# JunyiPeng00/wespeaker_hubert

Measured on AMD Instinct MI355X. Metric: embeddings/sec on 5s 16kHz utts, higher is better.
Workload: dtype f32 (bf16x3 split MFMA, fp32 accumulate)

## Files before the change

### wespeaker_hubert_amd/csrc/conv_gemm_x3_t6.hip

```cpp
#include "conv_gemm_x3_g.h"

namespace wsp {
namespace {

constexpr int kGCsLd = 68;
constexpr int kGCsBytes = 8 * 64 * kGCsLd * 4;
template <int ACT>
__device__ __forceinline__ void g_epilogue_cs(const ConvGemmArgs& p, f32x4 (&acc)[4][8], int m0, int n0, int wm,
                                              int wn, int wave, int lane, unsigned char* smem) {
  float* stg = reinterpret_cast<float*>(smem) + wave * 64 * kGCsLd;
  const int c16 = lane & 15, q = lane >> 4;
  const int cl = 4 * c16;
  const __amdgpu_buffer_rsrc_t ro = make_rsrc(p.out);
  const int nb = min((m0 / p.T + 1) * p.T, p.M) - m0, mb = p.M - m0;
  unsigned side0 = 0, side1 = 0;
#pragma unroll
  for (int k = 0; k < 16; ++k) {
    const int rr = wm * 64 + (k >> 2) * 16 + 4 * q + (k & 3);
    side0 |= (rr < nb ? 1u : 0u) << k;
    side1 |= (rr >= nb && rr < mb ? 1u : 0u) << k;
  }
  double rs[8][2];
#pragma unroll
  for (int pp = 0; pp < 2; ++pp) {
#pragma unroll
    for (int i = 0; i < 4; ++i)
#pragma unroll
      for (int jj = 0; jj < 4; ++jj)
#pragma unroll
        for (int r = 0; r < 4; ++r) stg[(16 * i + 4 * q + r) * kGCsLd + 16 * jj + c16] = acc[i][4 * pp + jj][r];
    asm volatile("s_waitcnt lgkmcnt(0)" ::: "memory");
    const int col = n0 + wn * 128 + 64 * pp + cl;
    const f32x4 bv = p.bias ? *reinterpret_cast<const f32x4*>(p.bias + col) : f32x4{0.f, 0.f, 0.f, 0.f};
    const f32x4 sc = p.scale ? *reinterpret_cast<const f32x4*>(p.scale + col) : f32x4{1.f, 1.f, 1.f, 1.f};
    const f32x4 sh = p.scale ? *reinterpret_cast<const f32x4*>(p.shift + col) : f32x4{0.f, 0.f, 0.f, 0.f};
#pragma unroll
    for (int u = 0; u < 16; ++u) {
      const int rl = 4 * u + q;
      const int row = m0 + wm * 64 + rl;
      float* sp = stg + rl * kGCsLd + cl;
      const f32x4 x = *reinterpret_cast<const f32x4*>(sp);
      f32x4 y;
#pragma unroll
      for (int e = 0; e < 4; ++e) {
        float v = x[e] + bv[e];
        if constexpr (ACT == kActRelu) v = fmaxf(v, 0.f);
        else if constexpr (ACT == kActTanh) v = tanhf(v);
        else if constexpr (ACT == kActGelu) v = gelu_as(v);
        y[e] = v * sc[e] + sh[e];
      }
      __builtin_amdgcn_raw_buffer_store_b128(__builtin_bit_cast(u32x4, y), ro,
                                             row < p.M ? (row * p.ldo + col) * 4 : kOOB, 0, 0);
      *reinterpret_cast<f32x4*>(sp) = y;
    }
    asm volatile("s_waitcnt lgkmcnt(0)" ::: "memory");
#pragma unroll
    for (int jj = 0; jj < 4; ++jj) {
      double c0 = 0.0, c1 = 0.0;
#pragma unroll
      for (int k = 0; k < 16; ++k) {
        const double yd = (double)stg[((k >> 2) * 16 + 4 * q + (k & 3)) * kGCsLd + 16 * jj + c16];
        c0 += (side0 >> k) & 1 ? yd : 0.0;
        c1 += (side1 >> k) & 1 ? yd : 0.0;
      }
      double v0 = c0 + __shfl_xor(c0, 16);
      v0 += __shfl_xor(v0, 32);
      double v1 = c1 + __shfl_xor(c1, 16);
      v1 += __shfl_xor(v1, 32);
      rs[4 * pp + jj][0] = v0;
      rs[4 * pp + jj][1] = v1;
      __builtin_amdgcn_sched_barrier(0);
    }
    asm volatile("s_waitcnt lgkmcnt(0)" ::: "memory");
  }
  __syncthreads();
  constexpr int BN = 256;
  double* red = reinterpret_cast<double*>(smem);
  if (lane < 16) {
#pragma unroll
    for (int j = 0; j < 8; ++j)
#pragma unroll
      for (int u = 0; u < 2; ++u) red[(wm * 2 + u) * BN + (wn * 8 + j) * 16 + lane] = rs[j][u];
  }
  __syncthreads();
  const int tid = threadIdx.x;
  if (tid < 2 * BN) {
    const int u = tid / BN, c = tid - u * BN;
    double v = 0.0;
#pragma unroll
    for (int w = 0; w < 4; ++w) v += red[(w * 2 + u) * BN + c];
    p.colsum[((size_t)(m0 / 256) * 2 + u) * p.N + n0 + c] = v;
  }
}

template <int AM, bool CSK, int LNM = 0>
__global__ __launch_bounds__(512, 1) void conv_gemm_g(const ConvGemmArgs p, const __bf16* __restrict__ whi,
                                                      const __bf16* __restrict__ wlo) {
  using L = Lds<true, 16>;
  constexpr bool DENSE = AM == 1 || AM == 3 || AM == 4;
  constexpr bool GATE = AM == 4;
  static_assert(!GATE || (!CSK && LNM == 0), "the gated instance: plain epilogues only");
  extern __shared__ __attribute__((aligned(16))) unsigned char smem[];
  const int tid = threadIdx.x;
  const int lane = tid & 63;
  const int wave = tid >> 6;
  const int ntiles = p.N / 256;
  const int mtiles = (p.M + 255) / 256;
  const int wg = xcd_remap(blockIdx.x, ntiles * mtiles);
  const int mt = wg / ntiles;
  const int nt = wg - mt * ntiles;
  const int m0 = mt * 256;
  const int n0 = nt * 256;

  const int ac0 = 4 * ((lane & 7) ^ ((lane >> 4) & 1)), ac1 = ac0 ^ 16;
  int a_r[4], a_t[DENSE ? 1 : 4], a_l[DENSE ? 1 : 4], a_s[AM == 3 ? 4 : 1];
#pragma unroll
  for (int i = 0; i < 4; ++i) {
    const int m = m0 + (4 * wave + i) * 8 + (lane >> 3);
    if constexpr (DENSE) {
      a_r[i] = m < p.M ? m : -1;
      if constexpr (AM == 3) {
        const int fto = p.Fo * p.To;
        const int b = m / fto, fo = (m - b * fto) / p.To, to = m - b * fto - fo * p.To;
        a_s[i] = m < p.M ? (b * p.Fi + fo * p.stride) * p.Ti + to * p.stride : -1;
      }
    } else if (p.seg) {
      const int mm = m < p.M ? m : p.M - 1;
      const int b = seg_of(p.seg, p.nseg, mm);
      const int t = (mm - p.seg[b]) * p.stride;
      const int* is = p.iseg ? p.iseg : p.seg;
      a_r[i] = is[b] + t;
      a_t[i] = (m < p.M) ? t : -0x40000000;
      a_l[i] = is[b + 1] - is[b];
    } else {
      const int b = m / p.T;
      const int t = (m - b * p.T) * p.stride;
      a_r[i] = b * p.Ti + t;
      a_t[i] = (m < p.M) ? t : -0x40000000;
      a_l[i] = p.Ti;
    }
  }
  int woff[2];
#pragma unroll
  for (int i = 0; i < 2; ++i) {
    const int row = (2 * wave + i) * 16 + (lane >> 2);
    const int c = (lane & 3) ^ ((0x1320 >> (4 * ((row >> 2) & 3))) & 3);
    woff[i] = ((n0 + row) * p.Kp + 8 * c) * 2;
  }
  const __amdgpu_buffer_rsrc_t rwh = make_rsrc(whi);
  const __amdgpu_buffer_rsrc_t rwl = make_rsrc(wlo);
  const int nk = p.Kp / BK;
  int jt = 0, ct = 0;
  auto dma = [&](int kt, int buf) {
    unsigned char* st = smem + buf * kGStage;
    const int off = jt * p.dil - p.pad;
    const float* base = p.a[0];
    int ld = p.lda[0], cl = ct;
    if (ct >= p.cseg[2]) {
      base = p.a[2];
      ld = p.lda[2];
      cl = ct - p.cseg[2];
    } else if (ct >= p.cseg[1]) {
      base = p.a[1];
      ld = p.lda[1];
      cl = ct - p.cseg[1];
    }
    const __amdgpu_buffer_rsrc_t ra = make_rsrc(base);
#pragma unroll
    for (int i = 0; i < 4; ++i) {
      if constexpr (DENSE) {
        const int ar = AM == 3 && ct >= p.cseg[1] ? a_s[i] : a_r[i];
        g_dma(ra, st + (4 * wave + i) * 1024, ar >= 0 ? (ar * ld + cl + (i & 1 ? ac1 : ac0)) * 4 : kOOB);
      } else if constexpr (AM == 2) {
        const int k = kt * BK + (i & 1 ? ac1 : ac0);
        const int tap = k / p.cin;
        const int offk = tap * p.dil - p.pad;
        const int tt = a_t[i] + offk;
        const bool ok = k < p.K && tt >= 0 && tt < a_l[i];
        g_dma(ra, st + (4 * wave + i) * 1024, ok ? ((a_r[i] + offk) * ld + k - tap * p.cin) * 4 : kOOB);
      } else {
        const int tt = a_t[i] + off;
        const bool ok = tt >= 0 && tt < a_l[i];
        g_dma(ra, st + (4 * wave + i) * 1024, ok ? ((a_r[i] + off) * ld + cl + (i & 1 ? ac1 : ac0)) * 4 : kOOB);
      }
    }
#pragma unroll
    for (int i = 0; i < 2; ++i) {
      const int o = woff[i] + kt * 64;
      g_dma(rwh, st + kGA + (2 * wave + i) * 1024, o);
      g_dma(rwl, st + kGA + kGW + (2 * wave + i) * 1024, o);
    }
    ct += 32;
    if (ct >= p.cin) {
      ct -= p.cin;
      ++jt;
    }
  };

  const int wm = wave >> 1, wn = wave & 1;
  const int r16 = lane & 15, qk = lane >> 4;
  f32x4 acc[4][8];
#pragma unroll
  for (int i = 0; i < 4; ++i)
#pragma unroll
    for (int j = 0; j < 8; ++j) acc[i][j] = f32x4{0.f, 0.f, 0.f, 0.f};
  bf16x8 ah[2], al[2], bh[4], bl[4];
  const int g_nb = GATE ? min((m0 / p.T + 1) * p.T, p.M) - m0 : 0;
  const int g_slot = GATE ? (p.K - p.gate_k0) * 4 : 0;
  auto rdA = [&](auto gated, const unsigned char* st, int ih, const unsigned char* gp = nullptr) {
#pragma clang fp contract(off)
#pragma unroll
    for (int i = 0; i < 2; ++i) {
      const int r = wm * 64 + (ih * 2 + i) * 16 + r16;
      f32x4 x0 = *reinterpret_cast<const f32x4*>(st + g_aslot(r, 2 * qk));
      f32x4 x1 = *reinterpret_cast<const f32x4*>(st + g_aslot(r, 2 * qk + 1));
      if constexpr (decltype(gated)::value) {
        const unsigned char* gr = gp + (r >= g_nb ? g_slot : 0);
        x0 = x0 * *reinterpret_cast<const f32x4*>(gr);
        x1 = x1 * *reinterpret_cast<const f32x4*>(gr + 16);
      }
#pragma unroll
      for (int e = 0; e < 4; ++e) {
        const __bf16 h0 = (__bf16)x0[e], h1 = (__bf16)x1[e];
        ah[i][e] = h0;
        ah[i][4 + e] = h1;
        al[i][e] = (__bf16)(x0[e] - (float)h0);
        al[i][4 + e] = (__bf16)(x1[e] - (float)h1);
      }
    }
  };
  auto rdB = [&](const unsigned char* st, int jh) {
#pragma unroll
    for (int j = 0; j < 4; ++j) {
      const int o = L::off(wn * 128 + (jh * 4 + j) * 16 + r16, qk * 16);
      bh[j] = *reinterpret_cast<const bf16x8*>(st + kGA + o);
      bl[j] = *reinterpret_cast<const bf16x8*>(st + kGA + kGW + o);
    }
  };
  auto mm = [&](int ih, int jh) {
#pragma unroll
    for (int i = 0; i < 2; ++i)
#pragma unroll
      for (int j = 0; j < 4; ++j) {
        f32x4& c = acc[ih * 2 + i][jh * 4 + j];
        c = __builtin_amdgcn_mfma_f32_16x16x32_bf16(al[i], bh[j], c, 0, 0, 0);
        c = __builtin_amdgcn_mfma_f32_16x16x32_bf16(ah[i], bl[j], c, 0, 0, 0);
        c = __builtin_amdgcn_mfma_f32_16x16x32_bf16(ah[i], bh[j], c, 0, 0, 0);
      }
  };

  float lmu = 0.f, lrs = 1.f;
  if constexpr ((LNM & 6) != 0) g_ln_row(p, min(m0 + wm * 64 + lane, p.M - 1), lmu, lrs);
  if constexpr (GATE) {
    const int ppu = g_slot >> 10, b0 = m0 / p.T;
    const __amdgpu_buffer_rsrc_t rg = make_rsrc(p.gate);
#pragma unroll
    for (int i = 0; i < 4; ++i) {
      const int q = 8 * i + wave;
      if (q >= 2 * ppu) break;
      const int u = q >= ppu ? 1 : 0;
      const bool ok = (b0 + u) * p.T < p.M;
      g_dma(rg, smem + 2 * kGStage + q * 1024, ok ? ((b0 + u) * p.ldg + (q - u * ppu) * 256 + lane * 4) * 4 : kOOB);
    }
  }
  dma(0, 0);
  dma(1, 1);
  asm volatile("s_waitcnt vmcnt(8)" ::: "memory");
  __builtin_amdgcn_s_barrier();
  auto ktile = [&](auto gated, int kt) {
    const int buf = kt & 1;
    const unsigned char* st = smem + buf * kGStage;
    const unsigned char* gp =
        decltype(gated)::value ? smem + 2 * kGStage + (kt * BK - p.gate_k0 + 8 * qk) * 4 : nullptr;
    rdA(gated, st, 0, gp);
    rdB(st, 0);
    mm(0, 0);
    rdB(st, 1);
    mm(0, 1);
    rdA(gated, st, 1, gp);
    mm(1, 1);
    rdB(st, 0);
    mm(1, 0);
    asm volatile("s_waitcnt vmcnt(0) lgkmcnt(0)" ::: "memory");
    __builtin_amdgcn_s_barrier();
    __builtin_amdgcn_sched_barrier(0);
    if (kt + 2 < nk) dma(kt + 2, buf);
  };
  const int ktg = GATE ? p.gate_k0 / BK : nk;
  for (int kt = 0; kt < ktg; ++kt) ktile(std::false_type{}, kt);
  if constexpr (GATE)
    for (int kt = ktg; kt < nk; ++kt) ktile(std::true_type{}, kt);
#define WSP_GEPI(RB, RES)                                                                                   \
  switch (p.act) {                                                                                         \
    case kActRelu: g_epilogue_rows<kActRelu, RB, RES>(p, acc, m0, n0, wm, wn, wave, lane, smem); break;    \
    case kActTanh: g_epilogue_rows<kActTanh, RB, RES>(p, acc, m0, n0, wm, wn, wave, lane, smem); break;    \
    case kActGelu: g_epilogue_rows<kActGelu, RB, RES>(p, acc, m0, n0, wm, wn, wave, lane, smem); break;    \
    default: g_epilogue_rows<kActNone, RB, RES>(p, acc, m0, n0, wm, wn, wave, lane, smem); break;          \
  }
  if constexpr (LNM != 0) {
    if constexpr ((LNM & 5) != 0)
      g_epilogue_rows<kActNone, false, true, LNM>(p, acc, m0, n0, wm, wn, wave, lane, smem, lmu, lrs);
    else if (p.act == kActGelu)
      g_epilogue_rows<kActGelu, false, false, LNM>(p, acc, m0, n0, wm, wn, wave, lane, smem, lmu, lrs);
    else
      g_epilogue_rows<kActNone, false, false, LNM>(p, acc, m0, n0, wm, wn, wave, lane, smem, lmu, lrs);
  } else if constexpr (CSK) {
    switch (p.act) {
      case kActRelu: g_epilogue_cs<kActRelu>(p, acc, m0, n0, wm, wn, wave, lane, smem); break;
      case kActTanh: g_epilogue_cs<kActTanh>(p, acc, m0, n0, wm, wn, wave, lane, smem); break;
      case kActGelu: g_epilogue_cs<kActGelu>(p, acc, m0, n0, wm, wn, wave, lane, smem); break;
      default: g_epilogue_cs<kActNone>(p, acc, m0, n0, wm, wn, wave, lane, smem); break;
    }
  } else if (p.res) {
    WSP_GEPI(false, true)
  } else if (p.row_bias) {
    WSP_GEPI(true, false)
  } else {
    WSP_GEPI(false, false)
  }
#undef WSP_GEPI
}

}

namespace x3 {

bool g256_supported(const ConvGemmArgs& p) {
  auto a16 = [](const void* q) { return (reinterpret_cast<uintptr_t>(q) & 15) == 0; };
  const bool aligned = a16(p.out) && p.ldo % 4 == 0 && a16(p.bias) && a16(p.scale) && a16(p.shift) &&
                       a16(p.row_bias) && a16(p.res) && (!p.res || p.ldres % 4 == 0);
  return aligned && p.N % 256 == 0 && !p.conv2d && !p.gcols && p.amode == kACat &&
         (uniform_ktiles(p) || (p.cseg[1] >= p.cin && !p.colsum)) &&
         (!p.sc2d || (uniform_ktiles(p) && !p.colsum && !p.lnmode && !p.row_bias));
}

bool g256_gate_supported(const ConvGemmArgs& p) {
  if (!p.gate || !g256_supported(p) || !uniform_ktiles(p)) return false;
  const bool dense = p.taps == 1 && p.pad == 0 && p.stride == 1 && !p.iseg && !p.seg && p.Ti == p.T;
  const int gk = p.K - p.gate_k0;
  return dense && p.T >= 256 && p.M % p.T == 0 && !p.colsum && !p.lnmode && !p.sc2d && p.K == p.Kp &&
         p.gate_k0 >= 0 && p.gate_k0 % 32 == 0 && gk > 0 && gk % 128 == 0 && gk <= 4096 && p.ldg >= gk &&
         p.ldg % 4 == 0 && (reinterpret_cast<uintptr_t>(p.gate) & 15) == 0 &&
         (long long)(p.M / p.T) * p.ldg * 4 < (long long)kOOB;
}

void t_g256(const ConvGemmArgs& p, const __bf16* h, const __bf16* l, hipStream_t s) {
  const int nwg = ((p.M + 255) / 256) * (p.N / 256);
  constexpr int lds0 = 2 * kGStage > kGEpiBytes ? 2 * kGStage : kGEpiBytes;
  constexpr int lds = lds0 > kGCsBytes ? lds0 : kGCsBytes;
  const bool dense = p.taps == 1 && p.pad == 0 && p.stride == 1 && !p.iseg && (p.seg || p.Ti == p.T);
  const int am = !uniform_ktiles(p) ? 2 : dense ? 1 : 0;
  if (p.gate) {
    WSP_CHECK(g256_gate_supported(p), "conv_gemm_x3: the gated A tail needs a dense 1x1 GEMM over a uniform batch");
    const int ldsg = std::max(lds, 2 * kGStage + 2 * (p.K - p.gate_k0) * 4);
    hipLaunchKernelGGL((conv_gemm_g<4, false>), dim3(nwg), dim3(512), ldsg, s, p, h, l);
    WSP_HIP(hipGetLastError());
    return;
  }
  if (p.sc2d) {
    hipLaunchKernelGGL((conv_gemm_g<3, false>), dim3(nwg), dim3(512), lds, s, p, h, l);
    WSP_HIP(hipGetLastError());
    return;
  }
  if (p.lnmode) {
    WSP_CHECK(am == 1 && !p.colsum && !p.row_bias && !p.scale && p.N % 128 == 0 &&
                  ((p.lnmode & 1) == 0 || (p.ln_out && p.res && p.act == kActNone)) &&
                  ((p.lnmode & 6) == 0 || (p.ln_in && p.ln_parts >= 1 && p.ln_parts <= kLnMaxParts)) && ((p.lnmode & 2) == 0 || (p.ln_cs && !p.res)) &&
                  (p.lnmode != 2 || p.act == kActNone || p.act == kActGelu) &&
                  ((p.lnmode & 4) == 0 || (p.ln_g && p.ln_b && p.res && p.act == kActNone)),
              "conv_gemm_x3: LayerNorm fold needs a dense 1x1 GEMM and its operands (fold: no activation or GELU)");
    switch (p.lnmode) {
      case 1: hipLaunchKernelGGL((conv_gemm_g<1, false, 1>), dim3(nwg), dim3(512), lds, s, p, h, l); break;
      case 2: hipLaunchKernelGGL((conv_gemm_g<1, false, 2>), dim3(nwg), dim3(512), lds, s, p, h, l); break;
      case 4: hipLaunchKernelGGL((conv_gemm_g<1, false, 4>), dim3(nwg), dim3(512), lds, s, p, h, l); break;
      case 5: hipLaunchKernelGGL((conv_gemm_g<1, false, 5>), dim3(nwg), dim3(512), lds, s, p, h, l); break;
      default: WSP_CHECK(false, "conv_gemm_x3: lnmode must be 1, 2, 4 or 5");
    }
    WSP_HIP(hipGetLastError());
    return;
  }
  if (p.colsum && am == 1)
    hipLaunchKernelGGL((conv_gemm_g<1, true>), dim3(nwg), dim3(512), lds, s, p, h, l);
  else if (p.colsum && am == 0)
    hipLaunchKernelGGL((conv_gemm_g<0, true>), dim3(nwg), dim3(512), lds, s, p, h, l);
  else if (am == 1)
    hipLaunchKernelGGL((conv_gemm_g<1, false>), dim3(nwg), dim3(512), lds, s, p, h, l);
  else if (am == 0)
    hipLaunchKernelGGL((conv_gemm_g<0, false>), dim3(nwg), dim3(512), lds, s, p, h, l);
  else
    hipLaunchKernelGGL((conv_gemm_g<2, false>), dim3(nwg), dim3(512), lds, s, p, h, l);
  WSP_HIP(hipGetLastError());
}

}
}
```

### wespeaker_hubert_amd/csrc/astp_fused.hip

```cpp
#include "astp_fused.h"
#include "gemm_common.h"

namespace wsp {

namespace {

typedef __bf16 bf16x8 __attribute__((ext_vector_type(8)));

constexpr int kK = 128;

typedef __attribute__((address_space(3))) void lds_void;

__device__ __forceinline__ void dma16(__amdgpu_buffer_rsrc_t r, unsigned char* lds, int voff) {
  __builtin_amdgcn_raw_ptr_buffer_load_lds(r, (lds_void*)lds, 16, voff, 0, 0, 0);
}

constexpr int kCB2 = 256;
constexpr int kChunkBytes = 32 * kK * 4;

constexpr int kLds3 = 3 * kChunkBytes;

__global__ __launch_bounds__(512, 1) void astp_fused3_kernel(const AstpArgs p) {
  extern __shared__ __attribute__((aligned(16))) unsigned char ring[];
  const int tid = threadIdx.x;
  const int lane = tid & 63;
  const int wave = tid >> 6;
  const int r32 = lane & 31;
  const int h = lane >> 5;
  const int nct = p.C / kCB2;
  const int id = xcd_remap(blockIdx.x, gridDim.x);
  const int b = id / nct;
  const int ct = id - b * nct;
  const int r0 = p.seg ? p.seg[b] : b * p.T;
  const int T = p.seg ? p.seg[b + 1] - r0 : p.T;
  const int col = ct * kCB2 + wave * 32 + r32;
  const __amdgpu_buffer_rsrc_t ra = make_rsrc(p.att + (size_t)r0 * kK);
  const __amdgpu_buffer_rsrc_t rx = make_rsrc(p.x + (size_t)r0 * p.ldx);

  auto dma_chunk = [&](int t0, int slot) {
#pragma unroll
    for (int j = 0; j < 2; ++j) {
      const int piece = 2 * wave + j;
      const int row = 2 * piece + h;
      const int c = r32 ^ (row & 15);
      const int t = t0 + row;
      dma16(ra, ring + slot * kChunkBytes + piece * 1024, t < T ? (t * kK + c * 4) * 4 : kOOB);
    }
  };
  auto load_x = [&](int t0, float (&xv)[16]) {
#pragma unroll
    for (int r = 0; r < 16; ++r) {
      const int t = t0 + (r & 3) + 8 * (r >> 2) + 4 * h;
      xv[r] = __builtin_bit_cast(float, __builtin_amdgcn_raw_buffer_load_b32(
                                            rx, t < T ? (t * p.ldx + col) * 4 : kOOB, 0, 0));
    }
  };
  bf16x8 wf[16];
  {
    const __amdgpu_buffer_rsrc_t rw = make_rsrc(p.w2);
    const int ntile = p.C / 32;
#pragma unroll
    for (int i = 0; i < 16; ++i)
      wf[i] = __builtin_bit_cast(bf16x8, __builtin_amdgcn_raw_buffer_load_b128(
                                             rw, ((i * ntile + ct * (kCB2 / 32) + wave) * 64 + lane) * 16, 0, 0));
  }
  const float bias = p.bias2[col];

  float m = -INFINITY, s = 0.f, a1 = 0.f, a2 = 0.f;
  auto consume = [&](int t0, int slot, const float (&xv)[16]) {
    const unsigned char* ab = ring + slot * kChunkBytes + r32 * 512;
    f32x16 acc;
#pragma unroll
    for (int r = 0; r < 16; ++r) acc[r] = 0.f;
#pragma unroll
    for (int ks = 0; ks < 8; ++ks) {
      const int c0 = 4 * ks + 2 * h;
      const f32x4 v0 = *reinterpret_cast<const f32x4*>(ab + ((c0 ^ (r32 & 15)) << 4));
      const f32x4 v1 = *reinterpret_cast<const f32x4*>(ab + (((c0 + 1) ^ (r32 & 15)) << 4));
      bf16x8 ah, al;
#pragma unroll
      for (int e = 0; e < 8; ++e) {
        const float v = e < 4 ? v0[e] : v1[e - 4];
        const __bf16 hh = (__bf16)v;
        ah[e] = hh;
        al[e] = (__bf16)(v - (float)hh);
      }
      acc = __builtin_amdgcn_mfma_f32_32x32x16_bf16(al, wf[2 * ks], acc, 0, 0, 0);
      acc = __builtin_amdgcn_mfma_f32_32x32x16_bf16(ah, wf[2 * ks + 1], acc, 0, 0, 0);
      acc = __builtin_amdgcn_mfma_f32_32x32x16_bf16(ah, wf[2 * ks], acc, 0, 0, 0);
    }
    float ev[16], mc = -INFINITY;
#pragma unroll
    for (int r = 0; r < 16; ++r) {
      const int t = t0 + (r & 3) + 8 * (r >> 2) + 4 * h;
      ev[r] = t < T ? acc[r] + bias : -INFINITY;
      mc = fmaxf(mc, ev[r]);
    }
    if (mc != -INFINITY) {
      const float m1 = fmaxf(m, mc);
      const float sc = __expf(m - m1);
      s *= sc;
      a1 *= sc;
      a2 *= sc;
#pragma unroll
      for (int r = 0; r < 16; ++r) {
        const float pe = __expf(ev[r] - m1);
        s += pe;
        a1 = fmaf(pe, xv[r], a1);
        a2 = fmaf(pe * xv[r], xv[r], a2);
      }
      m = m1;
    }
  };

  float xa[16], xb[16], xc[16];
  const int nch = (T + 31) / 32;
  dma_chunk(0, 0);
  load_x(0, xa);
  if (nch > 1) {
    dma_chunk(32, 1);
    load_x(32, xb);
  }
  auto step = [&](int c, int slot, const float (&xcur)[16], float (&xnext2)[16]) {
    if (c + 1 < nch)
      asm volatile("s_waitcnt vmcnt(18)" ::: "memory");
    else
      asm volatile("s_waitcnt vmcnt(0)" ::: "memory");
    __syncthreads();
    if (c + 2 < nch) {
      dma_chunk((c + 2) * 32, slot == 0 ? 2 : slot - 1);
      load_x((c + 2) * 32, xnext2);
    }
    consume(c * 32, slot, xcur);
  };
  for (int c = 0; c < nch; c += 3) {
    step(c, 0, xa, xc);
    if (c + 1 >= nch) break;
    step(c + 1, 1, xb, xa);
    if (c + 2 >= nch) break;
    step(c + 2, 2, xc, xb);
  }
  const float mo = __shfl_xor(m, 32), so = __shfl_xor(s, 32), a1o = __shfl_xor(a1, 32), a2o = __shfl_xor(a2, 32);
  const float M = fmaxf(m, mo);
  const float f0 = m == -INFINITY ? 0.f : __expf(m - M);
  const float f1 = mo == -INFINITY ? 0.f : __expf(mo - M);
  const float S = s * f0 + so * f1;
  const float A1 = a1 * f0 + a1o * f1;
  const float A2 = a2 * f0 + a2o * f1;
  if (h == 0) {
    const float mean = A1 / S;
    p.out[(size_t)b * 2 * p.C + col] = mean;
    p.out[(size_t)b * 2 * p.C + p.C + col] = sqrtf(fmaxf(A2 / S - mean * mean, p.var_floor));
  }
}

}

bool astp_fused_supported(int C, int K) { return K == kK && C > 0 && C % kCB2 == 0; }

void launch_astp_fused(const AstpArgs& p, hipStream_t s) {
  WSP_CHECK(astp_fused_supported(p.C, kK) && p.B > 0 && (p.seg || p.T > 0), "astp_fused: bad shape");
  WSP_CHECK(p.seg || (long long)p.T * p.ldx * 4 < (long long)kOOB, "astp_fused: utterance exceeds 2 GiB");
  hipLaunchKernelGGL(astp_fused3_kernel, dim3(p.B * (p.C / kCB2)), dim3(512), kLds3, s, p);
  WSP_HIP(hipGetLastError());
}

}
```

Baseline: 26350.

## Compute colsum epilogue from registers and reuse the shared row-store epilogue

The column-sum epilogue no longer stages accumulators through a per-wave LDS tile. Each lane now applies bias, activation and scale to its accumulator registers, reduces them in double, and writes the partials to a separate LDS reduction region. A per-wave uniform mode selects fully-first-segment, fully-second-segment or mixed row masks, so the common cases skip the per-element masking. The output store is delegated to the shared g_epilogue_rows path, and the LDS size grows only for the colsum launches. In exchange the activation is computed twice, once for the sums and once for the stores.

```diff
diff --git a/wespeaker_hubert_amd/csrc/conv_gemm_x3_t6.hip b/wespeaker_hubert_amd/csrc/conv_gemm_x3_t6.hip
--- a/wespeaker_hubert_amd/csrc/conv_gemm_x3_t6.hip
+++ b/wespeaker_hubert_amd/csrc/conv_gemm_x3_t6.hip
@@ -3,85 +3,79 @@
 namespace wsp {
 namespace {
 
-constexpr int kGCsLd = 68;
-constexpr int kGCsBytes = 8 * 64 * kGCsLd * 4;
+constexpr int kGCsRed = 4 * 2 * 256 * 8;
+constexpr int kGCsBytes = kGEpiBytes + kGCsRed;
+static_assert(kGCsBytes <= 160 * 1024, "family 7 CSK epilogue: LDS");
 template <int ACT>
 __device__ __forceinline__ void g_epilogue_cs(const ConvGemmArgs& p, f32x4 (&acc)[4][8], int m0, int n0, int wm,
                                               int wn, int wave, int lane, unsigned char* smem) {
-  float* stg = reinterpret_cast<float*>(smem) + wave * 64 * kGCsLd;
+  constexpr int BN = 256;
+  double* red = reinterpret_cast<double*>(smem + kGEpiBytes);
   const int c16 = lane & 15, q = lane >> 4;
-  const int cl = 4 * c16;
-  const __amdgpu_buffer_rsrc_t ro = make_rsrc(p.out);
   const int nb = min((m0 / p.T + 1) * p.T, p.M) - m0, mb = p.M - m0;
-  unsigned side0 = 0, side1 = 0;
-#pragma unroll
-  for (int k = 0; k < 16; ++k) {
-    const int rr = wm * 64 + (k >> 2) * 16 + 4 * q + (k & 3);
-    side0 |= (rr < nb ? 1u : 0u) << k;
-    side1 |= (rr >= nb && rr < mb ? 1u : 0u) << k;
-  }
-  double rs[8][2];
-#pragma unroll
-  for (int pp = 0; pp < 2; ++pp) {
-#pragma unroll
-    for (int i = 0; i < 4; ++i)
-#pragma unroll
-      for (int jj = 0; jj < 4; ++jj)
-#pragma unroll
-        for (int r = 0; r < 4; ++r) stg[(16 * i + 4 * q + r) * kGCsLd + 16 * jj + c16] = acc[i][4 * pp + jj][r];
-    asm volatile("s_waitcnt lgkmcnt(0)" ::: "memory");
-    const int col = n0 + wn * 128 + 64 * pp + cl;
-    const f32x4 bv = p.bias ? *reinterpret_cast<const f32x4*>(p.bias + col) : f32x4{0.f, 0.f, 0.f, 0.f};
-    const f32x4 sc = p.scale ? *reinterpret_cast<const f32x4*>(p.scale + col) : f32x4{1.f, 1.f, 1.f, 1.f};
-    const f32x4 sh = p.scale ? *reinterpret_cast<const f32x4*>(p.shift + col) : f32x4{0.f, 0.f, 0.f, 0.f};
-#pragma unroll
-    for (int u = 0; u < 16; ++u) {
-      const int rl = 4 * u + q;
-      const int row = m0 + wm * 64 + rl;
-      float* sp = stg + rl * kGCsLd + cl;
-      const f32x4 x = *reinterpret_cast<const f32x4*>(sp);
-      f32x4 y;
-#pragma unroll
-      for (int e = 0; e < 4; ++e) {
-        float v = x[e] + bv[e];
-        if constexpr (ACT == kActRelu) v = fmaxf(v, 0.f);
-        else if constexpr (ACT == kActTanh) v = tanhf(v);
-        else if constexpr (ACT == kActGelu) v = gelu_as(v);
-        y[e] = v * sc[e] + sh[e];
-      }
-      __builtin_amdgcn_raw_buffer_store_b128(__builtin_bit_cast(u32x4, y), ro,
-                                             row < p.M ? (row * p.ldo + col) * 4 : kOOB, 0, 0);
-      *reinterpret_cast<f32x4*>(sp) = y;
-    }
-    asm volatile("s_waitcnt lgkmcnt(0)" ::: "memory");
-#pragma unroll
-    for (int jj = 0; jj < 4; ++jj) {
-      double c0 = 0.0, c1 = 0.0;
-#pragma unroll
-      for (int k = 0; k < 16; ++k) {
-        const double yd = (double)stg[((k >> 2) * 16 + 4 * q + (k & 3)) * kGCsLd + 16 * jj + c16];
+  float bv[8], sc[8], sh[8];
+#pragma unroll
+  for (int j = 0; j < 8; ++j) {
+    const int col = n0 + wn * 128 + 16 * j + c16;
+    bv[j] = p.bias ? p.bias[col] : 0.f;
+    sc[j] = p.scale ? p.scale[col] : 1.f;
+    sh[j] = p.scale ? p.shift[col] : 0.f;
+  }
+  auto tile = [&](int j, auto mode, unsigned side0, unsigned side1) {
+    constexpr int MODE = decltype(mode)::value;
+    double c0 = 0.0, c1 = 0.0;
+#pragma unroll
+    for (int k = 0; k < 16; ++k) {
+      float v = acc[k >> 2][j][k & 3] + bv[j];
+      if constexpr (ACT == kActRelu) v = fmaxf(v, 0.f);
+      else if constexpr (ACT == kActTanh) v = tanhf(v);
+      else if constexpr (ACT == kActGelu) v = gelu_as(v);
+      const double yd = (double)(v * sc[j] + sh[j]);
+      if constexpr (MODE == 0) {
+        c0 += yd;
+      } else if constexpr (MODE == 1) {
+        c1 += yd;
+      } else {
         c0 += (side0 >> k) & 1 ? yd : 0.0;
         c1 += (side1 >> k) & 1 ? yd : 0.0;
       }
-      double v0 = c0 + __shfl_xor(c0, 16);
+    }
+    double v0 = 0.0, v1 = 0.0;
+    if constexpr (MODE != 1) {
+      v0 = c0 + __shfl_xor(c0, 16);
       v0 += __shfl_xor(v0, 32);
-      double v1 = c1 + __shfl_xor(c1, 16);
+    }
+    if constexpr (MODE != 0) {
+      v1 = c1 + __shfl_xor(c1, 16);
       v1 += __shfl_xor(v1, 32);
-      rs[4 * pp + jj][0] = v0;
-      rs[4 * pp + jj][1] = v1;
-      __builtin_amdgcn_sched_barrier(0);
-    }
-    asm volatile("s_waitcnt lgkmcnt(0)" ::: "memory");
-  }
-  __syncthreads();
-  constexpr int BN = 256;
-  double* red = reinterpret_cast<double*>(smem);
-  if (lane < 16) {
-#pragma unroll
-    for (int j = 0; j < 8; ++j)
-#pragma unroll
-      for (int u = 0; u < 2; ++u) red[(wm * 2 + u) * BN + (wn * 8 + j) * 16 + lane] = rs[j][u];
-  }
+    }
+    if (lane < 16) {
+      red[(wm * 2 + 0) * BN + (wn * 8 + j) * 16 + lane] = v0;
+      red[(wm * 2 + 1) * BN + (wn * 8 + j) * 16 + lane] = v1;
+    }
+    asm volatile("" ::: "memory");
+    __builtin_amdgcn_sched_barrier(0);
+  };
+  const int r0 = wm * 64;
+  const int wmode = __builtin_amdgcn_readfirstlane(r0 + 64 <= nb ? 0 : (r0 >= nb && r0 + 64 <= mb ? 1 : 2));
+  if (wmode == 0) {
+#pragma unroll
+    for (int j = 0; j < 8; ++j) tile(j, std::integral_constant<int, 0>{}, 0u, 0u);
+  } else if (wmode == 1) {
+#pragma unroll
+    for (int j = 0; j < 8; ++j) tile(j, std::integral_constant<int, 1>{}, 0u, 0u);
+  } else {
+    unsigned side0 = 0, side1 = 0;
+#pragma unroll
+    for (int k = 0; k < 16; ++k) {
+      const int rr = r0 + (k >> 2) * 16 + 4 * q + (k & 3);
+      side0 |= (rr < nb ? 1u : 0u) << k;
+      side1 |= (rr >= nb && rr < mb ? 1u : 0u) << k;
+    }
+#pragma unroll
+    for (int j = 0; j < 8; ++j) tile(j, std::integral_constant<int, 2>{}, side0, side1);
+  }
+  g_epilogue_rows<ACT, false, false>(p, acc, m0, n0, wm, wn, wave, lane, smem);
   __syncthreads();
   const int tid = threadIdx.x;
   if (tid < 2 * BN) {
@@ -347,7 +341,8 @@
 void t_g256(const ConvGemmArgs& p, const __bf16* h, const __bf16* l, hipStream_t s) {
   const int nwg = ((p.M + 255) / 256) * (p.N / 256);
   constexpr int lds0 = 2 * kGStage > kGEpiBytes ? 2 * kGStage : kGEpiBytes;
-  constexpr int lds = lds0 > kGCsBytes ? lds0 : kGCsBytes;
+  constexpr int lds = lds0;
+  constexpr int ldscs = lds0 > kGCsBytes ? lds0 : kGCsBytes;
   const bool dense = p.taps == 1 && p.pad == 0 && p.stride == 1 && !p.iseg && (p.seg || p.Ti == p.T);
   const int am = !uniform_ktiles(p) ? 2 : dense ? 1 : 0;
   if (p.gate) {
@@ -380,9 +375,9 @@
     return;
   }
   if (p.colsum && am == 1)
-    hipLaunchKernelGGL((conv_gemm_g<1, true>), dim3(nwg), dim3(512), lds, s, p, h, l);
+    hipLaunchKernelGGL((conv_gemm_g<1, true>), dim3(nwg), dim3(512), ldscs, s, p, h, l);
   else if (p.colsum && am == 0)
-    hipLaunchKernelGGL((conv_gemm_g<0, true>), dim3(nwg), dim3(512), lds, s, p, h, l);
+    hipLaunchKernelGGL((conv_gemm_g<0, true>), dim3(nwg), dim3(512), ldscs, s, p, h, l);
   else if (am == 1)
     hipLaunchKernelGGL((conv_gemm_g<1, false>), dim3(nwg), dim3(512), lds, s, p, h, l);
   else if (am == 0)
```

After: 26540 (median of 6 runs). No clear change (+0.7%).

## Pre-split attention rows into bf16 hi/lo LDS planes and pipeline split with MFMA

Applied to the files above, without the earlier changes.

Instead of every wave converting fp32 attention values into bf16 hi/lo pairs inside the MFMA loop, the kernel now splits each chunk once, cooperatively, into double-buffered bf16 planes in LDS. The split of chunk c+1 overlaps with the MFMAs of chunk c. Out-of-range handling moves from per-load index checks to buffer-descriptor byte limits, so loads past T return zero without branches. The wait counts are rewritten as tuned s_waitcnt sequences. This adds LDS footprint and relies on exact vmcnt accounting, including unconditional issue past the end of the utterance.

```diff
diff --git a/wespeaker_hubert_amd/csrc/astp_fused.hip b/wespeaker_hubert_amd/csrc/astp_fused.hip
--- a/wespeaker_hubert_amd/csrc/astp_fused.hip
+++ b/wespeaker_hubert_amd/csrc/astp_fused.hip
@@ -1,27 +1,43 @@
 #include "astp_fused.h"
+#include "bf16x3.h"
 #include "gemm_common.h"
 
 namespace wsp {
 
 namespace {
 
-typedef __bf16 bf16x8 __attribute__((ext_vector_type(8)));
-
 constexpr int kK = 128;
 
 typedef __attribute__((address_space(3))) void lds_void;
+
+__device__ __forceinline__ __amdgpu_buffer_rsrc_t rsrc_bytes(const void* base, unsigned bytes) {
+  const unsigned long long a = reinterpret_cast<unsigned long long>(base);
+  const unsigned lo = __builtin_amdgcn_readfirstlane((unsigned)a);
+  const unsigned hi = __builtin_amdgcn_readfirstlane((unsigned)(a >> 32));
+  void* p = reinterpret_cast<void*>(((unsigned long long)hi << 32) | lo);
+  return __builtin_amdgcn_make_buffer_rsrc(p, (short)0, (int)__builtin_amdgcn_readfirstlane(bytes), 0x00020000);
+}
 
 __device__ __forceinline__ void dma16(__amdgpu_buffer_rsrc_t r, unsigned char* lds, int voff) {
   __builtin_amdgcn_raw_ptr_buffer_load_lds(r, (lds_void*)lds, 16, voff, 0, 0, 0);
 }
 
+template <int VM, int LGKM = 15>
+__device__ __forceinline__ void wait_counts() {
+  asm volatile("" ::: "memory");
+  __builtin_amdgcn_s_waitcnt((VM & 15) | (7 << 4) | (LGKM << 8) | ((VM >> 4) << 14));
+  asm volatile("" ::: "memory");
+}
+
 constexpr int kCB2 = 256;
 constexpr int kChunkBytes = 32 * kK * 4;
-
-constexpr int kLds3 = 3 * kChunkBytes;
+constexpr int kPlaneBytes = 32 * kK * 2;
+
+constexpr int kLds3 = 3 * kChunkBytes + 4 * kPlaneBytes;
 
 __global__ __launch_bounds__(512, 1) void astp_fused3_kernel(const AstpArgs p) {
   extern __shared__ __attribute__((aligned(16))) unsigned char ring[];
+  unsigned char* const planes = ring + 3 * kChunkBytes;
   const int tid = threadIdx.x;
   const int lane = tid & 63;
   const int wave = tid >> 6;
@@ -34,8 +50,10 @@
   const int r0 = p.seg ? p.seg[b] : b * p.T;
   const int T = p.seg ? p.seg[b + 1] - r0 : p.T;
   const int col = ct * kCB2 + wave * 32 + r32;
-  const __amdgpu_buffer_rsrc_t ra = make_rsrc(p.att + (size_t)r0 * kK);
-  const __amdgpu_buffer_rsrc_t rx = make_rsrc(p.x + (size_t)r0 * p.ldx);
+  const __amdgpu_buffer_rsrc_t ra = rsrc_bytes(p.att + (size_t)r0 * kK, (unsigned)T * kK * 4u);
+  const __amdgpu_buffer_rsrc_t rx = rsrc_bytes(p.x + (size_t)r0 * p.ldx, (unsigned)T * (unsigned)p.ldx * 4u);
+  const unsigned ldx4 = (unsigned)p.ldx * 4u;
+  const unsigned xoff = 4u * h * ldx4 + 4u * col;
 
   auto dma_chunk = [&](int t0, int slot) {
 #pragma unroll
@@ -43,17 +61,29 @@
       const int piece = 2 * wave + j;
       const int row = 2 * piece + h;
       const int c = r32 ^ (row & 15);
-      const int t = t0 + row;
-      dma16(ra, ring + slot * kChunkBytes + piece * 1024, t < T ? (t * kK + c * 4) * 4 : kOOB);
+      dma16(ra, ring + slot * kChunkBytes + piece * 1024, (unsigned)t0 * (kK * 4u) + (row * kK + c * 4) * 4u);
     }
   };
   auto load_x = [&](int t0, float (&xv)[16]) {
 #pragma unroll
     for (int r = 0; r < 16; ++r) {
-      const int t = t0 + (r & 3) + 8 * (r >> 2) + 4 * h;
-      xv[r] = __builtin_bit_cast(float, __builtin_amdgcn_raw_buffer_load_b32(
-                                            rx, t < T ? (t * p.ldx + col) * 4 : kOOB, 0, 0));
-    }
+      const unsigned tr = (unsigned)(t0 + (r & 3) + 8 * (r >> 2));
+      xv[r] = __builtin_bit_cast(float, __builtin_amdgcn_raw_buffer_load_b32(rx, tr * ldx4 + xoff, 0, 0));
+    }
+  };
+  auto split_rows = [&](int slot, int pp) {
+    const int row = 4 * wave + (lane >> 4);
+    const int q = lane & 15;
+    const int sw = row & 15;
+    const unsigned char* src = ring + slot * kChunkBytes + row * 512;
+    const f32x4 v0 = *reinterpret_cast<const f32x4*>(src + (((2 * q) ^ sw) << 4));
+    const f32x4 v1 = *reinterpret_cast<const f32x4*>(src + (((2 * q + 1) ^ sw) << 4));
+    const float v[8] = {v0[0], v0[1], v0[2], v0[3], v1[0], v1[1], v1[2], v1[3]};
+    bf16x8 hi, lo;
+    split(v, hi, lo);
+    unsigned char* dst = planes + pp * 2 * kPlaneBytes + row * 256 + ((q ^ sw) << 4);
+    *reinterpret_cast<bf16x8*>(dst) = hi;
+    *reinterpret_cast<bf16x8*>(dst + kPlaneBytes) = lo;
   };
   bf16x8 wf[16];
   {
@@ -65,36 +95,36 @@
                                              rw, ((i * ntile + ct * (kCB2 / 32) + wave) * 64 + lane) * 16, 0, 0));
   }
   const float bias = p.bias2[col];
+  asm volatile("" ::: "memory");
 
   float m = -INFINITY, s = 0.f, a1 = 0.f, a2 = 0.f;
-  auto consume = [&](int t0, int slot, const float (&xv)[16]) {
-    const unsigned char* ab = ring + slot * kChunkBytes + r32 * 512;
-    f32x16 acc;
+  auto multiply = [&](int pp, f32x16& acc) {
+    const unsigned char* ab = planes + pp * 2 * kPlaneBytes + r32 * 256;
 #pragma unroll
     for (int r = 0; r < 16; ++r) acc[r] = 0.f;
 #pragma unroll
     for (int ks = 0; ks < 8; ++ks) {
-      const int c0 = 4 * ks + 2 * h;
-      const f32x4 v0 = *reinterpret_cast<const f32x4*>(ab + ((c0 ^ (r32 & 15)) << 4));
-      const f32x4 v1 = *reinterpret_cast<const f32x4*>(ab + (((c0 + 1) ^ (r32 & 15)) << 4));
-      bf16x8 ah, al;
-#pragma unroll
-      for (int e = 0; e < 8; ++e) {
-        const float v = e < 4 ? v0[e] : v1[e - 4];
-        const __bf16 hh = (__bf16)v;
-        ah[e] = hh;
-        al[e] = (__bf16)(v - (float)hh);
+      const int o = ((2 * ks + h) ^ (r32 & 15)) << 4;
+      const bf16x8 ah = *reinterpret_cast<const bf16x8*>(ab + o);
+      const bf16x8 al = *reinterpret_cast<const bf16x8*>(ab + kPlaneBytes + o);
+      mma3(ah, al, wf[2 * ks], wf[2 * ks + 1], acc);
+    }
+  };
+  auto update = [&](int t0, const f32x16& acc, const float (&xv)[16]) {
+    float ev[16], mc = -INFINITY;
+    if (t0 + 32 <= T) {
+#pragma unroll
+      for (int r = 0; r < 16; ++r) {
+        ev[r] = acc[r] + bias;
+        mc = fmaxf(mc, ev[r]);
       }
-      acc = __builtin_amdgcn_mfma_f32_32x32x16_bf16(al, wf[2 * ks], acc, 0, 0, 0);
-      acc = __builtin_amdgcn_mfma_f32_32x32x16_bf16(ah, wf[2 * ks + 1], acc, 0, 0, 0);
-      acc = __builtin_amdgcn_mfma_f32_32x32x16_bf16(ah, wf[2 * ks], acc, 0, 0, 0);
-    }
-    float ev[16], mc = -INFINITY;
-#pragma unroll
-    for (int r = 0; r < 16; ++r) {
-      const int t = t0 + (r & 3) + 8 * (r >> 2) + 4 * h;
-      ev[r] = t < T ? acc[r] + bias : -INFINITY;
-      mc = fmaxf(mc, ev[r]);
+    } else {
+#pragma unroll
+      for (int r = 0; r < 16; ++r) {
+        const int t = t0 + (r & 3) + 8 * (r >> 2) + 4 * h;
+        ev[r] = t < T ? acc[r] + bias : -INFINITY;
+        mc = fmaxf(mc, ev[r]);
+      }
     }
     if (mc != -INFINITY) {
       const float m1 = fmaxf(m, mc);
@@ -115,23 +145,26 @@
 
   float xa[16], xb[16], xc[16];
   const int nch = (T + 31) / 32;
-  dma_chunk(0, 0);
-  load_x(0, xa);
-  if (nch > 1) {
-    dma_chunk(32, 1);
-    load_x(32, xb);
-  }
+  auto issue = [&](int t0, int slot, float (&xv)[16]) {
+    dma_chunk(t0, slot);
+    asm volatile("" ::: "memory");
+    load_x(t0, xv);
+    asm volatile("" ::: "memory");
+  };
+  issue(0, 0, xa);
+  issue(32, 1, xb);
+  wait_counts<34>();
+  split_rows(0, 0);
   auto step = [&](int c, int slot, const float (&xcur)[16], float (&xnext2)[16]) {
-    if (c + 1 < nch)
-      asm volatile("s_waitcnt vmcnt(18)" ::: "memory");
-    else
-      asm volatile("s_waitcnt vmcnt(0)" ::: "memory");
-    __syncthreads();
-    if (c + 2 < nch) {
-      dma_chunk((c + 2) * 32, slot == 0 ? 2 : slot - 1);
-      load_x((c + 2) * 32, xnext2);
-    }
-    consume(c * 32, slot, xcur);
+    wait_counts<18, 0>();
+    __builtin_amdgcn_s_barrier();
+    asm volatile("" ::: "memory");
+    issue((c + 2) * 32, slot == 0 ? 2 : slot - 1, xnext2);
+    f32x16 acc;
+    multiply(c & 1, acc);
+    wait_counts<34>();
+    split_rows(slot == 2 ? 0 : slot + 1, (c + 1) & 1);
+    update(c * 32, acc, xcur);
   };
   for (int c = 0; c < nch; c += 3) {
     step(c, 0, xa, xc);
@@ -140,6 +173,7 @@
     if (c + 2 >= nch) break;
     step(c + 2, 2, xc, xb);
   }
+  wait_counts<0>();
   const float mo = __shfl_xor(m, 32), so = __shfl_xor(s, 32), a1o = __shfl_xor(a1, 32), a2o = __shfl_xor(a2, 32);
   const float M = fmaxf(m, mo);
   const float f0 = m == -INFINITY ? 0.f : __expf(m - M);
```

After: 26320 before, 26550 after (median of 6 runs). About the same (+0.9%).
